# NVIDIA/tensorrt-laboratory

Hardware: NVIDIA H100
Metric: ResNet-50 fp16 b=8 inferences/sec (higher is better)
Workload: dtype f16

## Files before the change

tensorrt_laboratory_b200/csrc/engine.cu:

```cuda
#include <cuda.h>
#include <cuda_runtime.h>
#include <stdarg.h>
#include <stdio.h>
#include <stdlib.h>
#include <string.h>

#include <algorithm>
#include <map>
#include <memory>
#include <mutex>
#include <string>
#include <vector>

#include "../../include/b200infer.h"
#include "kernels.h"
#include "plan_format.h"

#include "b2_internal.h"

namespace b2i {
thread_local std::string g_err;
int fail(int code, const char* fmt, ...) {
    char buf[1024];
    va_list ap;
// ... 697 lines not shown
        const int tiles = m_tiles * (cout_phys / bn);
        for (int splits = 1; splits <= 8; ++splits) {
            if (honor_forced && c->force_splits && !group_span ? splits != c->force_splits : splits != 1) continue;
            if (splits > 1 && (kb != 64 || kblocks / splits < 4 || tiles * splits > 160 || tiles > kMaxSplitTiles ||
                               size_t(tiles) * splits * 128 * bn * 4 > kSplitWorkspaceBytes))
                continue;
            const int kpc = (kblocks + splits - 1) / splits;
            if (splits > 1 && (splits - 1) * kpc >= kblocks) continue;
            for (int st : stgs) {
                if (!b2k::conv_config_exists(bn, kb, st)) continue;
                if (b2k::conv_smem_bytes(bn, st, residual) > kSmemLimit) continue;
                if (honor_forced && c->force_stages && st != c->force_stages) continue;
                if (!(honor_forced && c->force_stages) && !stage_depth_useful(bn, kb, st, kpc)) continue;
                const double smem = b2k::conv_smem_bytes(bn, st, residual);
                int per_sm = int(double(kSmemLimit) / smem);
                per_sm = std::min(per_sm, bn <= 64 ? 2 : 1);
                per_sm = std::max(1, std::min(per_sm, 8));
                const int ctas = tiles * splits;
                const int waves = (ctas + g_sms * per_sm - 1) / (g_sms * per_sm);
                const int sharing = std::max(1, std::min(per_sm, (ctas + g_sms - 1) / g_sms));
                const double stage_bytes = 16384.0 + bn * 128.0;
                const double t_kb = std::max(stage_bytes / (70000.0 / sharing), 1.0 / st);
                double t_epi = 0.6 + bn / 64.0 * 0.4 + (residual ? 0.4 : 0.0);
                if (splits > 1) t_epi += 1.0 + 0.3 * splits;
                const double t_cta = 2.0 + kpc * t_kb + t_epi;
                double total = waves * t_cta;
                const double traffic = double(ctas) * kpc * stage_bytes;
                total = std::max(total, traffic / 5.0e6 + 2.0);
                if (total < best.est_us) best = ConvConfig{bn, st, splits, total};
            }
        }
// ... 1767 lines not shown
```

tensorrt_laboratory_b200/csrc/kernels.cu:

```cuda
#include "kernels.h"

#include <stdio.h>
#include <stdlib.h>
#include <string.h>

#include "ptx_sm90.cuh"
#include "wgmma_sm90.cuh"

namespace b2k {

template <int BN, int STAGES, int SPS = 1>
struct ConvCfg {
    static constexpr int A_SUBBLK = 128 * 64 * 2;
    static constexpr int B_SUBBLK = BN * 64 * 2;
    static constexpr int A_STAGE = SPS * A_SUBBLK;
    static constexpr int B_STAGE = SPS * B_SUBBLK;
    static constexpr int PIPE_BYTES = STAGES * (A_STAGE + B_STAGE);
    static constexpr int TILE_BYTES = 128 * BN * 2;
    static_assert(TILE_BYTES <= PIPE_BYTES, "the output staging tile reuses the pipeline buffers");
};

__host__ __device__ constexpr int conv_smem_layout_bytes(int bn, int stages, bool residual, int sps = 1) {
    return stages * sps * (128 * 64 * 2 + bn * 64 * 2) + (residual ? 128 * bn * 2 : 0) + 256 + bn * 4 + 1024;
}

constexpr int kConvThreads = 384;
constexpr int kConsumerWarps = 8;

struct FragPos {
    int row0, col0;
    __device__ FragPos(int consumer_warp, int lane)
        : row0(64 * (consumer_warp >> 2) + 16 * (consumer_warp & 3) + (lane >> 2)), col0(2 * (lane & 3)) {}
};

template <int BN, int KB, int STAGES, int SPS, int CN = 1, bool DBG = false, int AV = 0, bool GELU = false>
__global__ void __launch_bounds__(kConvThreads, BN <= 64 ? 2 : 1)
conv_f16_tcgen05(const __grid_constant__ CUtensorMap mapA, const __grid_constant__ CUtensorMap mapB,
                 const __grid_constant__ CUtensorMap mapOut, const __grid_constant__ CUtensorMap mapRes,
                 const ConvArgs p) {
    static_assert(SPS == 1 || KB == 64, "multi-sub-block stages exist for the 64-wide K path only");
    using Cfg = ConvCfg<BN, STAGES, SPS>;
    constexpr int TPS = 64 / KB;
    constexpr int A_SUB = 128 * KB * 2;
    constexpr int B_SUB = BN * KB * 2;
    constexpr int OW = BN >= 64 ? 64 : 32;
    constexpr int OROWB = OW * 2;
    constexpr int NBOX = BN / OW;

    extern __shared__ uint8_t smem_raw[];
    uint8_t* smem = smem_raw + ((1024u - (smem_u32(smem_raw) & 1023u)) & 1023u);
    const bool has_res = p.residual != nullptr;
    uint8_t* sA = smem;
    uint8_t* sB = smem + STAGES * Cfg::A_STAGE;
    uint8_t* sOut = smem;
    uint8_t* sRes = smem + Cfg::PIPE_BYTES;
    uint8_t* tail = sRes + (has_res ? Cfg::TILE_BYTES : 0);
// ... 37 lines not shown
    if (threadIdx.x == 0) {
        tma_prefetch_desc(&mapA);
        tma_prefetch_desc(&mapB);
        tma_prefetch_desc(&mapOut);
        if (has_res) tma_prefetch_desc(&mapRes);
        for (int s = 0; s < STAGES; ++s) {
            mbar_init(&full_bar[s], 1);
            mbar_init(&empty_bar[s], static_cast<uint32_t>(kConsumerWarps * cn));
        }
        mbar_init(res_bar, 1);
        fence_barrier_init();
        fence_proxy_async();
    }
    __syncthreads();
    if (cn > 1) cluster_sync_all();
    if (warp == 3) {
#pragma unroll
        for (int i = 0; i < BN / 32; ++i) s_bias[lane + 32 * i] = __ldg(p.bias + n0 + lane + 32 * i);
    }
    if (p.pdl_trigger == 0) pdl_launch_dependents();
    if (dbg && threadIdx.x == 0) dbg[1] = clock64();

    auto sub_tiles = [&](int kb) -> int {
        if (KB == 64) return 1;
        const int n = p.taps_phys - kb * TPS;
        return n > TPS ? TPS : n;
    };
    const bool skip_a = DBG && KB == 64 && (p.dbg_mode & 2), skip_b = DBG && KB == 64 && (p.dbg_mode & 4);
    auto stage_bytes = [&](int kb) -> uint32_t {
        if (KB == 64) {
            const int ns = subs_in_step((kb - kb_begin) / SPS);
            return static_cast<uint32_t>(ns * ((skip_a ? 0 : Cfg::A_SUBBLK) + (skip_b ? 0 : Cfg::B_SUBBLK)));
        }
        return static_cast<uint32_t>(sub_tiles(kb) * (A_SUB + B_SUB));
    };
    auto load_b = [&](int kb, int s) {
// ... 8 lines not shown
                } else {
                    tma_load_2d(&mapB, &full_bar[s], b_dst + u * Cfg::B_SUBBLK, (kb + u) * 64, n0);
                }
            }
        } else {
            const int nt = sub_tiles(kb);
            for (int t = 0; t < nt; ++t) tma_load_2d(&mapB, &full_bar[s], b_dst + t * B_SUB, (kb * TPS + t) * KB, n0);
        }
    };
    auto load_residual = [&]() {
        mbar_expect_tx(res_bar, Cfg::TILE_BYTES);
#pragma unroll
        for (int b = 0; b < NBOX; ++b) tma_load_2d(&mapRes, res_bar, sRes + b * (128 * OROWB), n0 + b * OW, m0);
    };

    if (warp == 0) {
        {
            int img0 = 0, p0 = 0, q0 = 0;
            const int slice_rows = 128 / cn;
            int ms = m0 + static_cast<int>(crank) * slice_rows;
            const uint32_t slice_off = crank * static_cast<uint32_t>(slice_rows) * 128u;
            if (!a_tiled) {
                if (ms >= p.M) ms = 0;
                img0 = ms / p.HoWo;
                const int rem = ms - img0 * p.HoWo;
                p0 = rem / p.Wo;
                q0 = rem - p0 * p.Wo;
            }
            const int base_w = q0 * p.stride_w - p.pad_w;
            const int base_h = p0 * p.stride_h - p.pad_h;
            int cur_cb = 0, cur_r = 0, cur_sx = 0;
            int cb0 = 0;
// ... 68 lines not shown
                if (dbg) c0 = clock64();
                mbar_wait(&empty_bar[s], ph ^ 1);
                if (dbg) c1 = clock64();
                if (elect_one_sync()) {
                    mbar_expect_tx(&full_bar[s], stage_bytes(kb_begin + i * SPS));
                    load_a(kb_begin + i * SPS, s);
                    if (!kSplitProducers) load_b(kb_begin + i * SPS, s);
                }
                __syncwarp();
                if (dbg) {
                    c3 = clock64();
                    tw += c1 - c0, tl += c3 - c1;
                }
            }
            if (dbg && lane == 0) dbg[11] = tw, dbg[12] = te, dbg[13] = tl;
        }
        __syncwarp();
    }

    const int cw = warp - 4;
    float acc[BN / 2];
    if (warp >= 4) {
        const uint32_t wg = static_cast<uint32_t>(cw >> 2);
        auto release_stage = [&](int st) {
            __syncwarp();
            if (lane == 0) {
                if (cn > 1) {
                    for (uint32_t r = 0; r < static_cast<uint32_t>(cn); ++r) mbar_arrive_cluster(&empty_bar[st], r);
                } else {
                    mbar_arrive(&empty_bar[st]);
                }
            }
        };
        long long mw = 0, mi = 0;
        for (int i = 0; i < nk; ++i) {
            const int s = i % STAGES;
            const uint32_t ph = (i / STAGES) & 1;
            long long m0c = 0, m1c = 0;
            if (dbg) m0c = clock64();
            mbar_wait(&full_bar[s], ph);
            if (dbg) m1c = clock64(), mw += m1c - m0c;
            if (dbg && i == 0 && cw == 0 && lane == 0) dbg[3] = clock64();
            const uint32_t a_addr = smem_u32(sA + s * Cfg::A_STAGE);
            const uint32_t b_addr = smem_u32(sB + s * Cfg::B_STAGE);
            if constexpr (KB == 64) {
                auto mma = [&](int t) {
                    const int u = t >> 2, j = t & 3;
                    const uint64_t ad = make_wgmma_desc(a_addr + u * Cfg::A_SUBBLK + wg * 8192 + j * 32, 16, 1024, WG_SW128);
                    const uint64_t bd = make_wgmma_desc(b_addr + u * Cfg::B_SUBBLK + j * 32, 16, 1024, WG_SW128);
                    wgmma_f16<BN>(acc, ad, bd, (i > 0 || t > 0) ? 1u : 0u);
                };
                if (SPS == 1 || subs_in_step(i) == SPS) wgmma_group<4 * SPS>(mma);
                else wgmma_group<4>(mma);
            } else if constexpr (KB == 32) {
                auto mma = [&](int t) {
                    const int st = t >> 1, j = t & 1;
                    const uint64_t ad = make_wgmma_desc(a_addr + st * A_SUB + wg * 4096 + j * 32, 16, 512, WG_SW64);
                    const uint64_t bd = make_wgmma_desc(b_addr + st * B_SUB + j * 32, 16, 512, WG_SW64);
                    wgmma_f16<BN>(acc, ad, bd, (i > 0 || t > 0) ? 1u : 0u);
                };
                if (sub_tiles(kb_begin + i) == TPS) wgmma_group<2 * TPS>(mma);
                else wgmma_group<2>(mma);
            } else {
                auto mma = [&](int j) {
                    const uint64_t ad = make_wgmma_desc(a_addr + 2 * j * A_SUB + wg * 1024, A_SUB, 128, WG_NOSWZ);
                    const uint64_t bd = make_wgmma_desc(b_addr + 2 * j * B_SUB, B_SUB, 128, WG_NOSWZ);
                    wgmma_f16<BN>(acc, ad, bd, (i > 0 || j > 0) ? 1u : 0u);
                };
                wgmma_group_upto<TPS / 2>(sub_tiles(kb_begin + i) / 2, mma);
            }
            if constexpr (STAGES == 1) {
                wgmma_wait<0>();
                release_stage(0);
            } else {
                wgmma_wait<1>();
                if (i > 0) release_stage((i - 1) % STAGES);
            }
            if (dbg) mi += clock64() - m1c;
        }
        if constexpr (STAGES > 1) {
            wgmma_wait<0>();
            if (nk > 0) release_stage((nk - 1) % STAGES);
        }
        if (dbg && cw == 0 && lane == 0) dbg[4] = clock64(), dbg[14] = mw, dbg[15] = mi;
    }

    if (warp == 3 && KB == 64) {
        for (int i = 0; i < nk; ++i) {
            const int s = i % STAGES;
            if (i >= STAGES) mbar_wait(&empty_bar[s], ((i / STAGES) & 1) ^ 1);
            if (elect_one_sync()) load_b(kb_begin + i * SPS, s);
            __syncwarp();
        }
    }

    pdl_wait();
    __syncthreads();
    if (dbg && threadIdx.x == 128) dbg[5] = clock64();
    if (p.pdl_trigger == 1) pdl_launch_dependents();
    const FragPos fp(cw, lane);

    auto finish_pair = [&](int row, int col, float v0, float v1) {
        const int box = col / OW;
        const int chunk = (col % OW) / 8;
        const uint32_t so = static_cast<uint32_t>(box * (128 * OROWB)) + swz_off<OROWB>(row, chunk) + (col % 8) * 2;
        v0 += s_bias[col];
        v1 += s_bias[col + 1];
        if (has_res) {
            const float2 rf = __half22float2(*reinterpret_cast<const __half2*>(sRes + so));
            v0 += rf.x;
            v1 += rf.y;
        }
        if constexpr (GELU) {
            v0 = gelu_erf(v0);
            v1 = gelu_erf(v1);
        } else if (p.relu) {
            v0 = fmaxf(v0, 0.0f);
            v1 = fmaxf(v1, 0.0f);
        }
        *reinterpret_cast<__half2*>(sOut + so) = __floats2half2_rn(v0, v1);
    };

    bool do_store = true;
    if (!split) {
        if (warp >= 4) {
            if (has_res) mbar_wait(res_bar, 0);
#pragma unroll
            for (int j = 0; j < BN / 8; ++j)
#pragma unroll
                for (int h = 0; h < 2; ++h) finish_pair(fp.row0 + 8 * h, 8 * j + fp.col0, acc[4 * j + 2 * h], acc[4 * j + 2 * h + 1]);
        }
    } else {
        const int tile = blockIdx.y * gridDim.x + blockIdx.x;
        float* ws_tile = p.workspace + static_cast<size_t>(tile) * p.splits * (128 * BN);
        if (warp >= 4) {
            float* mine = ws_tile + static_cast<size_t>(blockIdx.z) * (128 * BN);
#pragma unroll
            for (int j = 0; j < BN / 8; ++j)
#pragma unroll
                for (int h = 0; h < 2; ++h)
                    __stcg(reinterpret_cast<float2*>(mine + (fp.row0 + 8 * h) * BN + 8 * j + fp.col0),
                           make_float2(acc[4 * j + 2 * h], acc[4 * j + 2 * h + 1]));
        }
        __syncthreads();
        if (threadIdx.x == 0) {
            __threadfence();
            const int prev = atomicAdd(p.tile_counters + tile, 1);
            const uint32_t last = (prev == p.splits - 1) ? 1u : 0u;
            if (last) {
                p.tile_counters[tile] = 0;
                if (has_res) load_residual();
            }
            *last_flag = last;
        }
        __syncthreads();
        do_store = *last_flag != 0;
        if (do_store && warp >= 4) {
            __threadfence();
            if (has_res) mbar_wait(res_bar, 0);
#pragma unroll 4
            for (int j = 0; j < BN / 8; ++j) {
#pragma unroll
                for (int h = 0; h < 2; ++h) {
                    const int row = fp.row0 + 8 * h, col = 8 * j + fp.col0;
                    float f0 = 0.f, f1 = 0.f;
                    for (int sp = 0; sp < p.splits; ++sp) {
                        const float2 t = __ldcg(reinterpret_cast<const float2*>(ws_tile + static_cast<size_t>(sp) * (128 * BN) + row * BN + col));
                        f0 += t.x;
                        f1 += t.y;
                    }
                    finish_pair(row, col, f0, f1);
                }
            }
        }
    }
    if (dbg && threadIdx.x == 128) dbg[6] = clock64();
    if (p.pdl_trigger == 2) pdl_launch_dependents();
    fence_proxy_async();
    __syncthreads();
    if (threadIdx.x == 0 && do_store) {
#pragma unroll
        for (int b = 0; b < NBOX; ++b) tma_store_2d(&mapOut, sOut + b * (128 * OROWB), n0 + b * OW, m0);
        tma_store_commit_and_wait_read();
    }
    if (cn > 1) {
        if (warp == 1) {
            const int first = nk > STAGES ? nk - STAGES : 0;
            for (int i = first; i < nk; ++i) mbar_wait(&empty_bar[i % STAGES], (i / STAGES) & 1);
        }
        __syncthreads();
        cluster_sync_all();
    }
    if (dbg && threadIdx.x == 128) {
        dbg[7] = clock64();
        unsigned long long gt;
        asm volatile("mov.u64 %0, %%globaltimer;" : "=l"(gt));
        dbg[9] = static_cast<long long>(gt);
    }
}

__host__ __device__ constexpr int conv_ws_smem_bytes(int bn, int stages, int sps, bool residual) {
    return stages * sps * (128 * 64 * 2 + bn * 64 * 2) + 2 * 128 * bn * 2 + (residual ? 2 * 128 * bn * 2 : 0) + 256 + 1024;
}

template <int BN, int STAGES, int SPS>
__global__ void __launch_bounds__(kConvThreads, 1)
conv_f16_tcgen05_ws(const __grid_constant__ CUtensorMap mapA, const __grid_constant__ CUtensorMap mapOut,
                    const __grid_constant__ CUtensorMap mapRes, const ConvArgs p) {
    constexpr int A_SUBBLK = 128 * 64 * 2;
    constexpr int B_SUBBLK = BN * 64 * 2;
    constexpr int A_STAGE = SPS * A_SUBBLK;
    constexpr int B_STAGE = SPS * B_SUBBLK;
// ... 220 lines not shown
}

constexpr int kHaloMaxCBlocks = 8;
__host__ __device__ constexpr int halo_b_stages(int bn) { return bn >= 256 ? 3 : 4; }
__host__ __device__ constexpr int halo_a_stage_bytes(int w, int r) {
    const int loaded = (r + 2) * (w + 2);
    const int touched = 128 + 2 * (w + 2) + 2;
    const int rows = loaded > touched ? loaded : touched;
    return (rows * 128 + 1023) / 1024 * 1024;
}
__host__ __device__ constexpr int halo_smem_bytes(int bn, int w, int r, int cblocks) {
    return cblocks * halo_a_stage_bytes(w, r) + halo_b_stages(bn) * bn * 128 + 256 + bn * 4 + 1024;
}

template <int BN>
__global__ void __launch_bounds__(kConvThreads, 1)
conv3x3_halo_tcgen05(const __grid_constant__ CUtensorMap mapIn, const __grid_constant__ CUtensorMap mapOut, const ConvArgs p) {
    constexpr int NB = halo_b_stages(BN);
    constexpr int B_BLK = BN * 128;
    constexpr int OW = 64;
    constexpr int NBOX = BN / OW;

    extern __shared__ uint8_t smem_raw[];
    uint8_t* smem = smem_raw + ((1024u - (smem_u32(smem_raw) & 1023u)) & 1023u);
    const int W = p.Wo, Wp = p.Wo + 2, R = p.halo_rows;
    const int a_stage = halo_a_stage_bytes(W, R);
    const int cblocks = p.cblocks;
    uint8_t* sA = smem;
    uint8_t* sB = smem + cblocks * a_stage;
    uint8_t* sOut = smem;
    uint8_t* tail = sB + NB * B_BLK;
    uint64_t* a_full = reinterpret_cast<uint64_t*>(tail);
    uint64_t* b_full = a_full + kHaloMaxCBlocks;
// ... 12 lines not shown
    if (threadIdx.x == 0) {
        tma_prefetch_desc(&mapIn);
        tma_prefetch_desc(&mapOut);
        for (int s = 0; s < cblocks; ++s) mbar_init(&a_full[s], 1);
        for (int s = 0; s < NB; ++s) {
            mbar_init(&b_full[s], 1);
            mbar_init(&b_empty[s], kConsumerWarps);
        }
        fence_barrier_init();
        fence_proxy_async();
    }
    __syncthreads();
    if (p.pdl_trigger == 0) pdl_launch_dependents();

    float acc[BN / 2];
    if (warp == 0) {
        const uint32_t halo_bytes = static_cast<uint32_t>((R + 2) * Wp * 128);
        pdl_wait();
        if (elect_one_sync()) {
            for (int cb = 0; cb < cblocks; ++cb) {
                mbar_expect_tx(&a_full[cb], halo_bytes);
                tma_load_4d(&mapIn, &a_full[cb], sA + cb * a_stage, cb * 64, -1, h0 - 1, img);
            }
        }
        __syncwarp();
    } else if (warp >= 4) {
        const uint32_t wg_off = static_cast<uint32_t>((warp - 4) >> 2) * 8192u;
        int i = 0;
#pragma unroll 1
        for (int tap = 0; tap < 9; ++tap) {
            const int r = tap / 3, sx = tap - r * 3;
            const uint32_t tap_off = static_cast<uint32_t>((r * Wp + sx) * 128);
#pragma unroll 1
            for (int cb = 0; cb < cblocks; ++cb, ++i) {
                const int sb = i % NB;
                if (tap == 0) mbar_wait(&a_full[cb], 0);
                mbar_wait(&b_full[sb], (i / NB) & 1);
                const uint32_t a_addr = smem_u32(sA + cb * a_stage) + tap_off + wg_off;
                const uint32_t b_addr = smem_u32(sB + sb * B_BLK);
                wgmma_fence();
#pragma unroll
                for (int j = 0; j < 4; ++j) {
                    const uint64_t ad = make_wgmma_desc(a_addr + j * 32, 16, 1024, WG_SW128);
                    const uint64_t bd = make_wgmma_desc(b_addr + j * 32, 16, 1024, WG_SW128);
                    wgmma_f16<BN>(acc, ad, bd, (i > 0 || j > 0) ? 1u : 0u);
                }
                wgmma_commit();
                wgmma_wait<1>();
                __syncwarp();
                if (i > 0 && lane == 0) mbar_arrive(&b_empty[(i - 1) % NB]);
            }
        }
        wgmma_wait<0>();
        __syncwarp();
        if (lane == 0) mbar_arrive(&b_empty[(nsteps - 1) % NB]);
    } else if (warp == 3) {
        for (int i = lane; i < BN; i += 32) s_bias[i] = __ldg(p.bias + n0 + i);
        for (int i = 0; i < nsteps; ++i) {
            const int sb = i % NB;
            if (i >= NB) mbar_wait(&b_empty[sb], ((i / NB) & 1) ^ 1);
            if (elect_one_sync()) {
                mbar_expect_tx(&b_full[sb], B_BLK);
                bulk_load_1d(&b_full[sb], sB + sb * B_BLK, p.wpacked + (static_cast<size_t>(i) * (p.Cout >> 5) + (n0 >> 5)) * 4096,
                             B_BLK);
            }
            __syncwarp();
        }
    }

    pdl_wait();
    __syncthreads();
    if (p.pdl_trigger == 1) pdl_launch_dependents();
    if (warp >= 4) {
        const FragPos fp(warp - 4, lane);
#pragma unroll
        for (int j = 0; j < BN / 8; ++j) {
#pragma unroll
            for (int h = 0; h < 2; ++h) {
                const int row = fp.row0 + 8 * h, col = 8 * j + fp.col0;
                const uint32_t so = static_cast<uint32_t>((col / OW) * (128 * 128)) + swz_off<128>(row, (col % OW) / 8) + (col % 8) * 2;
                float v0 = acc[4 * j + 2 * h] + s_bias[col], v1 = acc[4 * j + 2 * h + 1] + s_bias[col + 1];
                if (p.relu) {
                    v0 = fmaxf(v0, 0.0f);
                    v1 = fmaxf(v1, 0.0f);
                }
                *reinterpret_cast<__half2*>(sOut + so) = __floats2half2_rn(v0, v1);
            }
        }
    }
    fence_proxy_async();
    __syncthreads();
    if (threadIdx.x == 0) {
#pragma unroll
        for (int b = 0; b < NBOX; ++b) tma_store_4d(&mapOut, sOut + b * (128 * 128), n0 + b * OW, 0, h0, img);
        tma_store_commit_and_wait_read();
    }
}

static bool g_use_pdl = true;
void set_pdl(bool on) { g_use_pdl = on; }
bool get_pdl() { return g_use_pdl; }

template <typename Kern, typename... Args>
static int launch_kernel_cluster(Kern kern, dim3 grid, dim3 block, size_t smem, cudaStream_t stream, bool pdl, unsigned cluster_x,
                                 Args... args) {
    cudaLaunchConfig_t cfg = {};
    cfg.gridDim = grid;
    cfg.blockDim = block;
    cfg.dynamicSmemBytes = smem;
    cfg.stream = stream;
// ... 58 lines not shown
                                                      cudaFuncAttributeMaxDynamicSharedMemorySize, bytes));
        if (e) return e;
        if constexpr (KB == 64) {
            if ((e = static_cast<int>(cudaFuncSetAttribute(conv_f16_tcgen05<BN, KB, STAGES, SPS, 1, false, 1>,
                                                           cudaFuncAttributeMaxDynamicSharedMemorySize, bytes)))) return e;
            if ((e = static_cast<int>(cudaFuncSetAttribute(conv_f16_tcgen05<BN, KB, STAGES, SPS, 1, false, 2>,
                                                           cudaFuncAttributeMaxDynamicSharedMemorySize, bytes)))) return e;
            if ((e = static_cast<int>(cudaFuncSetAttribute(conv_f16_tcgen05<BN, KB, STAGES, SPS, 1, false, 2, true>,
                                                           cudaFuncAttributeMaxDynamicSharedMemorySize, bytes)))) return e;
        }
    }
    return static_cast<int>(cudaFuncSetAttribute(conv_f16_tcgen05<BN, KB, STAGES, SPS, CN>, cudaFuncAttributeMaxDynamicSharedMemorySize, bytes));
}

int conv_smem_bytes(int bn, int stages, bool residual, int sps) { return conv_smem_layout_bytes(bn, stages, residual, sps); }

#define B2_FOR_EACH_CONV(X) \
    X(32, 64, 1, 1) X(32, 64, 2, 1) X(32, 64, 4, 1) X(32, 64, 8, 1) \
    X(64, 64, 1, 1) X(64, 64, 2, 1) X(64, 64, 4, 1) X(64, 64, 8, 1) \
    X(128, 64, 1, 1) X(128, 64, 2, 1) X(128, 64, 4, 1) X(256, 64, 2, 1) X(256, 64, 4, 1) \
    X(32, 64, 2, 2) X(32, 64, 4, 2) X(64, 64, 2, 2) X(64, 64, 4, 2) X(128, 64, 2, 2) X(256, 64, 2, 2) \
    X(32, 8, 2, 1) X(32, 8, 4, 1) X(64, 8, 2, 1) X(64, 8, 4, 1) X(64, 8, 8, 1) X(128, 8, 4, 1) \
    X(32, 32, 2, 1) X(32, 32, 4, 1) X(64, 32, 1, 1) X(64, 32, 2, 1) X(64, 32, 4, 1) X(128, 32, 2, 1) X(128, 32, 4, 1)

int conv_halo_smem(int bn, int w, int r, int cblocks) { return halo_smem_bytes(bn, w, r, cblocks); }
bool conv_halo_config_exists(int bn) { return bn == 64 || bn == 128 || bn == 256; }
static int init_conv_halo_kernels() {
    int e;
    if ((e = static_cast<int>(cudaFuncSetAttribute(conv3x3_halo_tcgen05<64>, cudaFuncAttributeMaxDynamicSharedMemorySize, 227 * 1024)))) return e;
    if ((e = static_cast<int>(cudaFuncSetAttribute(conv3x3_halo_tcgen05<128>, cudaFuncAttributeMaxDynamicSharedMemorySize, 227 * 1024)))) return e;
// ... 906 lines not shown
```

tensorrt_laboratory_b200/csrc/kernels.h:

```cpp
#pragma once
#include <cuda.h>
#include <cuda_fp16.h>
#include <cuda_runtime.h>
#include <stdint.h>

namespace b2k {

enum { A_TILED = 0, A_IM2COL = 1 };

struct ConvArgs {
    const float* bias;
    const __half* residual;
    __half* out;
    int M;
    int Cout;
    int num_kblocks;
    int cblocks;
    int taps;
    int taps_phys;
    int kw;
    int HoWo, Wo;
    int stride_h, stride_w;
    int pad_h, pad_w;
    int relu;
// ... 20 lines not shown
    ConvArgs args;
    int bn;
    int kb;
    int stages;
    int sps;
    int grid_m, grid_n;
    int cn;
    int halo;
    int ws_ctas;
};

int launch_conv_f16_tcgen05(const ConvLaunch& L, cudaStream_t stream);
int init_conv_kernels();
bool conv_config_exists(int bn, int kb, int stages, int sps = 1);
int conv_smem_bytes(int bn, int stages, bool residual, int sps = 1);
bool conv_cluster_config_exists(int bn, int stages, int sps, int cn);
bool conv_halo_config_exists(int bn);
int conv_halo_smem(int bn, int w, int r, int cblocks);
bool conv_ws_config_exists(int bn, int stages, int sps);
int conv_ws_smem(int bn, int stages, int sps, bool residual);
void set_pdl(bool on);
bool get_pdl();

constexpr int kNetMaxLayers = 160;

struct NetLayerInfo {
    const uint8_t* wpacked;
    const float* bias;
    __half* out;
    const __half* residual;
// ... 129 lines not shown
```

tensorrt_laboratory_b200/csrc/ptx_sm90.cuh:

```cuda
#pragma once
#include <cuda.h>
#include <cuda_fp16.h>
#include <cuda_runtime.h>
#include <stdint.h>

namespace b2k {

__device__ __forceinline__ uint32_t smem_u32(const void* p) {
    return static_cast<uint32_t>(__cvta_generic_to_shared(p));
}

__device__ __forceinline__ void mbar_init(uint64_t* bar, uint32_t count) {
    asm volatile("mbarrier.init.shared::cta.b64 [%0], %1;" ::"r"(smem_u32(bar)), "r"(count) : "memory");
}

__device__ __forceinline__ void mbar_expect_tx(uint64_t* bar, uint32_t bytes) {
    asm volatile("mbarrier.arrive.expect_tx.shared::cta.b64 _, [%0], %1;" ::"r"(smem_u32(bar)), "r"(bytes)
                 : "memory");
}

__device__ __forceinline__ uint32_t mbar_try_wait(uint64_t* bar, uint32_t parity) {
    uint32_t ok;
    asm volatile(
        "{\n"
        ".reg .pred p;\n"
        "mbarrier.try_wait.parity.shared::cta.b64 p, [%1], %2;\n"
        "selp.u32 %0, 1, 0, p;\n"
        "}\n"
        : "=r"(ok)
        : "r"(smem_u32(bar)), "r"(parity)
        : "memory");
    return ok;
}

__device__ __forceinline__ void mbar_wait(uint64_t* bar, uint32_t parity) {
    uint32_t spins = 0;
    long long t0 = 0;
    while (!mbar_try_wait(bar, parity)) {
        if ((++spins & 0x3FFFu) == 0) {
            long long now = clock64();
            if (t0 == 0) t0 = now;
            else if (now - t0 > 4000000000LL) __trap();
        }
    }
}

__device__ __forceinline__ bool elect_one_sync() {
    uint32_t pred;
    asm volatile(
        "{\n"
        ".reg .pred P;\n"
        "elect.sync _|P, 0xffffffff;\n"
        "selp.u32 %0, 1, 0, P;\n"
        "}\n"
        : "=r"(pred));
    return pred != 0;
}
// ... 79 lines not shown
}
__device__ __forceinline__ void tma_store_commit() { asm volatile("cp.async.bulk.commit_group;" ::: "memory"); }
__device__ __forceinline__ void tma_store_wait_read0() { asm volatile("cp.async.bulk.wait_group.read 0;" ::: "memory"); }
__device__ __forceinline__ void tma_store_wait_read1() { asm volatile("cp.async.bulk.wait_group.read 1;" ::: "memory"); }
__device__ __forceinline__ void tma_store_commit_and_wait_read() {
    asm volatile("cp.async.bulk.commit_group;" ::: "memory");
    asm volatile("cp.async.bulk.wait_group.read 0;" ::: "memory");
}

template <int ROWB>
__device__ __forceinline__ uint32_t swz_off(int row, int chunk) {
    if (ROWB == 128) return static_cast<uint32_t>(row * 128 + ((chunk ^ (row & 7)) << 4));
    return static_cast<uint32_t>(row * 64 + ((chunk ^ ((row >> 1) & 3)) << 4));
}

__device__ __forceinline__ void named_bar_sync(uint32_t id, uint32_t nthreads) {
    asm volatile("bar.sync %0, %1;" ::"r"(id), "r"(nthreads) : "memory");
}
__device__ __forceinline__ void mbar_arrive(uint64_t* bar) {
    asm volatile("mbarrier.arrive.shared::cta.b64 _, [%0];" ::"r"(smem_u32(bar)) : "memory");
}

__device__ __forceinline__ void tma_load_4d(const CUtensorMap* map, uint64_t* bar, void* dst, int c0, int c1, int c2, int c3) {
    asm volatile(
        "cp.async.bulk.tensor.4d.shared::cluster.global.mbarrier::complete_tx::bytes [%0], [%1, {%3, %4, %5, %6}], [%2];"
        ::"r"(smem_u32(dst)), "l"(reinterpret_cast<uint64_t>(map)), "r"(smem_u32(bar)), "r"(c0), "r"(c1), "r"(c2), "r"(c3)
        : "memory");
}
__device__ __forceinline__ void tma_store_4d(const CUtensorMap* map, const void* src, int c0, int c1, int c2, int c3) {
    asm volatile("cp.async.bulk.tensor.4d.global.shared::cta.bulk_group [%0, {%2, %3, %4, %5}], [%1];" ::"l"(
// ... 7 lines not shown
```

tensorrt_laboratory_b200/csrc/wgmma_sm90.cuh:

```cuda
#pragma once
#include <stdint.h>

namespace b2k {

__device__ __forceinline__ void wgmma_fence() { asm volatile("wgmma.fence.sync.aligned;" ::: "memory"); }
__device__ __forceinline__ void wgmma_commit() { asm volatile("wgmma.commit_group.sync.aligned;" ::: "memory"); }
template <int N>
__device__ __forceinline__ void wgmma_wait() { asm volatile("wgmma.wait_group.sync.aligned %0;" ::"n"(N) : "memory"); }

enum { WG_NOSWZ = 0, WG_SW128 = 1, WG_SW64 = 2 };
__device__ __forceinline__ uint64_t make_wgmma_desc(uint32_t saddr, uint32_t lbo_bytes, uint32_t sbo_bytes, uint32_t layout) {
    uint64_t d = 0;
    d |= static_cast<uint64_t>((saddr >> 4) & 0x3FFF);
    d |= static_cast<uint64_t>((lbo_bytes >> 4) & 0x3FFF) << 16;
    d |= static_cast<uint64_t>((sbo_bytes >> 4) & 0x3FFF) << 32;
    d |= static_cast<uint64_t>(layout & 3) << 62;
    return d;
}

__device__ __forceinline__ void wgmma_f16_n32(float (&d)[16], uint64_t a, uint64_t b, uint32_t accumulate) {
    asm volatile(
        "{\n.reg .pred p;\nsetp.ne.b32 p, %18, 0;\n"
        "wgmma.mma_async.sync.aligned.m64n32k16.f32.f16.f16 {%0, %1, %2, %3, %4, %5, %6, %7, %8, %9, %10, %11, %12, %13, %14, %15}, %16, %17, p, 1, 1, 0, 0;\n}\n"
        : "+f"(d[0]), "+f"(d[1]), "+f"(d[2]), "+f"(d[3]), "+f"(d[4]), "+f"(d[5]), "+f"(d[6]), "+f"(d[7]), "+f"(d[8]), "+f"(d[9]), "+f"(d[10]), "+f"(d[11]), "+f"(d[12]), "+f"(d[13]), "+f"(d[14]), "+f"(d[15])
// ... 43 lines not shown
}
__device__ __forceinline__ void wgmma_i8_n256(int32_t (&d)[128], uint64_t a, uint64_t b, uint32_t accumulate) {
    asm volatile(
        "{\n.reg .pred p;\nsetp.ne.b32 p, %130, 0;\n"
        "wgmma.mma_async.sync.aligned.m64n256k32.s32.s8.s8 {%0, %1, %2, %3, %4, %5, %6, %7, %8, %9, %10, %11, %12, %13, %14, %15, %16, %17, %18, %19, %20, %21, %22, %23, %24, %25, %26, %27, %28, %29, %30, %31, %32, %33, %34, %35, %36, %37, %38, %39, %40, %41, %42, %43, %44, %45, %46, %47, %48, %49, %50, %51, %52, %53, %54, %55, %56, %57, %58, %59, %60, %61, %62, %63, %64, %65, %66, %67, %68, %69, %70, %71, %72, %73, %74, %75, %76, %77, %78, %79, %80, %81, %82, %83, %84, %85, %86, %87, %88, %89, %90, %91, %92, %93, %94, %95, %96, %97, %98, %99, %100, %101, %102, %103, %104, %105, %106, %107, %108, %109, %110, %111, %112, %113, %114, %115, %116, %117, %118, %119, %120, %121, %122, %123, %124, %125, %126, %127}, %128, %129, p;\n}\n"
        : "+r"(d[0]), "+r"(d[1]), "+r"(d[2]), "+r"(d[3]), "+r"(d[4]), "+r"(d[5]), "+r"(d[6]), "+r"(d[7]), "+r"(d[8]), "+r"(d[9]), "+r"(d[10]), "+r"(d[11]), "+r"(d[12]), "+r"(d[13]), "+r"(d[14]), "+r"(d[15]), "+r"(d[16]), "+r"(d[17]), "+r"(d[18]), "+r"(d[19]), "+r"(d[20]), "+r"(d[21]), "+r"(d[22]), "+r"(d[23]), "+r"(d[24]), "+r"(d[25]), "+r"(d[26]), "+r"(d[27]), "+r"(d[28]), "+r"(d[29]), "+r"(d[30]), "+r"(d[31]), "+r"(d[32]), "+r"(d[33]), "+r"(d[34]), "+r"(d[35]), "+r"(d[36]), "+r"(d[37]), "+r"(d[38]), "+r"(d[39]), "+r"(d[40]), "+r"(d[41]), "+r"(d[42]), "+r"(d[43]), "+r"(d[44]), "+r"(d[45]), "+r"(d[46]), "+r"(d[47]), "+r"(d[48]), "+r"(d[49]), "+r"(d[50]), "+r"(d[51]), "+r"(d[52]), "+r"(d[53]), "+r"(d[54]), "+r"(d[55]), "+r"(d[56]), "+r"(d[57]), "+r"(d[58]), "+r"(d[59]), "+r"(d[60]), "+r"(d[61]), "+r"(d[62]), "+r"(d[63]), "+r"(d[64]), "+r"(d[65]), "+r"(d[66]), "+r"(d[67]), "+r"(d[68]), "+r"(d[69]), "+r"(d[70]), "+r"(d[71]), "+r"(d[72]), "+r"(d[73]), "+r"(d[74]), "+r"(d[75]), "+r"(d[76]), "+r"(d[77]), "+r"(d[78]), "+r"(d[79]), "+r"(d[80]), "+r"(d[81]), "+r"(d[82]), "+r"(d[83]), "+r"(d[84]), "+r"(d[85]), "+r"(d[86]), "+r"(d[87]), "+r"(d[88]), "+r"(d[89]), "+r"(d[90]), "+r"(d[91]), "+r"(d[92]), "+r"(d[93]), "+r"(d[94]), "+r"(d[95]), "+r"(d[96]), "+r"(d[97]), "+r"(d[98]), "+r"(d[99]), "+r"(d[100]), "+r"(d[101]), "+r"(d[102]), "+r"(d[103]), "+r"(d[104]), "+r"(d[105]), "+r"(d[106]), "+r"(d[107]), "+r"(d[108]), "+r"(d[109]), "+r"(d[110]), "+r"(d[111]), "+r"(d[112]), "+r"(d[113]), "+r"(d[114]), "+r"(d[115]), "+r"(d[116]), "+r"(d[117]), "+r"(d[118]), "+r"(d[119]), "+r"(d[120]), "+r"(d[121]), "+r"(d[122]), "+r"(d[123]), "+r"(d[124]), "+r"(d[125]), "+r"(d[126]), "+r"(d[127])
        : "l"(a), "l"(b), "r"(accumulate));
}
template <int N>
__device__ __forceinline__ void wgmma_f16(float (&d)[N / 2], uint64_t a, uint64_t b, uint32_t accumulate) {
    if constexpr (N == 32) wgmma_f16_n32(d, a, b, accumulate);
    else if constexpr (N == 64) wgmma_f16_n64(d, a, b, accumulate);
    else if constexpr (N == 128) wgmma_f16_n128(d, a, b, accumulate);
    else wgmma_f16_n256(d, a, b, accumulate);
}
template <int N>
__device__ __forceinline__ void wgmma_i8(int32_t (&d)[N / 2], uint64_t a, uint64_t b, uint32_t accumulate) {
    if constexpr (N == 32) wgmma_i8_n32(d, a, b, accumulate);
    else if constexpr (N == 64) wgmma_i8_n64(d, a, b, accumulate);
    else if constexpr (N == 128) wgmma_i8_n128(d, a, b, accumulate);
    else wgmma_i8_n256(d, a, b, accumulate);
}

template <int N, class F>
__device__ __forceinline__ void wgmma_group(F&& mma) {
    wgmma_fence();
#pragma unroll
    for (int t = 0; t < N; ++t) mma(t);
    wgmma_commit();
}
// ... 13 lines not shown
```

Before: 29970.

## Rebalance warpgroup registers with setmaxnreg and allow two CTAs per SM for BN=128

Producer warpgroups now give up registers with setmaxnreg.dec and consumer warpgroups take more with setmaxnreg.inc, so accumulators can fit when launch bounds ask for two CTAs per SM. BN=128 conv kernels, and BN<=64 halo kernels, get min-blocks 2 when shared memory allows. The host cost model now uses the same CTAs-per-SM rule. When registers are tight, the wgmma N dimension is split into column blocks. The epilogue is moved into a per-role lambda and some barrier waits drop the trap path. The risks are register spills in the consumer warps, and extra wgmma instructions when N is split.

Measured after the change: 30830 (median of 6 runs). +2.9%, better.

```diff
diff --git a/tensorrt_laboratory_b200/csrc/engine.cu b/tensorrt_laboratory_b200/csrc/engine.cu
--- a/tensorrt_laboratory_b200/csrc/engine.cu
+++ b/tensorrt_laboratory_b200/csrc/engine.cu
@@ -735,7 +735,7 @@
                 if (!(honor_forced && c->force_stages) && !stage_depth_useful(bn, kb, st, kpc)) continue;
                 const double smem = b2k::conv_smem_bytes(bn, st, residual);
                 int per_sm = int(double(kSmemLimit) / smem);
-                per_sm = std::min(per_sm, bn <= 64 ? 2 : 1);
+                per_sm = std::min(per_sm, b2k::conv_regs_ctas_per_sm(bn, st));
                 per_sm = std::max(1, std::min(per_sm, 8));
                 const int ctas = tiles * splits;
                 const int waves = (ctas + g_sms * per_sm - 1) / (g_sms * per_sm);
diff --git a/tensorrt_laboratory_b200/csrc/kernels.cu b/tensorrt_laboratory_b200/csrc/kernels.cu
--- a/tensorrt_laboratory_b200/csrc/kernels.cu
+++ b/tensorrt_laboratory_b200/csrc/kernels.cu
@@ -3,6 +3,8 @@
 #include <stdio.h>
 #include <stdlib.h>
 #include <string.h>
+
+#include <type_traits>
 
 #include "ptx_sm90.cuh"
 #include "wgmma_sm90.cuh"
@@ -27,6 +29,19 @@
 constexpr int kConvThreads = 384;
 constexpr int kConsumerWarps = 8;
 
+template <int BN, int MinBlocks>
+struct ConvRegs {
+    static constexpr int kLaunch = 65536 / (kConvThreads * MinBlocks) / 8 * 8;
+    static constexpr int kProducer = 40;
+    static constexpr int kConsumer = (kConvThreads * kLaunch - 128 * kProducer) / 256 / 8 * 8;
+    static constexpr int kMmaN = BN / 2 + 26 <= kLaunch ? BN : 64;
+    static_assert(128 * kProducer + 256 * kConsumer <= kConvThreads * kLaunch, "setmaxnreg.inc would wait forever");
+    static_assert(kConsumer <= 256 && BN / 2 + 32 <= kConsumer, "setmaxnreg range, accumulators");
+};
+__host__ __device__ constexpr int conv_min_blocks(int bn, int stages, int sps) {
+    return bn <= 64 || (bn == 128 && 2 * (conv_smem_layout_bytes(bn, stages, true, sps) + 1024) <= 228 * 1024) ? 2 : 1;
+}
+
 struct FragPos {
     int row0, col0;
     __device__ FragPos(int consumer_warp, int lane)
@@ -34,12 +49,13 @@
 };
 
 template <int BN, int KB, int STAGES, int SPS, int CN = 1, bool DBG = false, int AV = 0, bool GELU = false>
-__global__ void __launch_bounds__(kConvThreads, BN <= 64 ? 2 : 1)
+__global__ void __launch_bounds__(kConvThreads, conv_min_blocks(BN, STAGES, SPS))
 conv_f16_tcgen05(const __grid_constant__ CUtensorMap mapA, const __grid_constant__ CUtensorMap mapB,
                  const __grid_constant__ CUtensorMap mapOut, const __grid_constant__ CUtensorMap mapRes,
                  const ConvArgs p) {
     static_assert(SPS == 1 || KB == 64, "multi-sub-block stages exist for the 64-wide K path only");
     using Cfg = ConvCfg<BN, STAGES, SPS>;
+    using Regs = ConvRegs<BN, conv_min_blocks(BN, STAGES, SPS)>;
     constexpr int TPS = 64 / KB;
     constexpr int A_SUB = 128 * KB * 2;
     constexpr int B_SUB = BN * KB * 2;
@@ -107,12 +123,6 @@
     }
     __syncthreads();
     if (cn > 1) cluster_sync_all();
-    if (warp == 3) {
-#pragma unroll
-        for (int i = 0; i < BN / 32; ++i) s_bias[lane + 32 * i] = __ldg(p.bias + n0 + lane + 32 * i);
-    }
-    if (p.pdl_trigger == 0) pdl_launch_dependents();
-    if (dbg && threadIdx.x == 0) dbg[1] = clock64();
 
     auto sub_tiles = [&](int kb) -> int {
         if (KB == 64) return 1;
@@ -151,8 +161,125 @@
         for (int b = 0; b < NBOX; ++b) tma_load_2d(&mapRes, res_bar, sRes + b * (128 * OROWB), n0 + b * OW, m0);
     };
 
-    if (warp == 0) {
-        {
+    const int cw = warp - 4;
+    float acc[BN / 2];
+
+    auto epilogue = [&](auto role) {
+        constexpr bool kConsumer = decltype(role)::value;
+        pdl_wait();
+        __syncthreads();
+        if (kConsumer && dbg && threadIdx.x == 128) dbg[5] = clock64();
+        if (p.pdl_trigger == 1) pdl_launch_dependents();
+        const FragPos fp(cw, lane);
+
+        auto finish_pair = [&](int row, int col, float v0, float v1) {
+            const int box = col / OW;
+            const int chunk = (col % OW) / 8;
+            const uint32_t so = static_cast<uint32_t>(box * (128 * OROWB)) + swz_off<OROWB>(row, chunk) + (col % 8) * 2;
+            v0 += s_bias[col];
+            v1 += s_bias[col + 1];
+            if (has_res) {
+                const float2 rf = __half22float2(*reinterpret_cast<const __half2*>(sRes + so));
+                v0 += rf.x;
+                v1 += rf.y;
+            }
+            if constexpr (GELU) {
+                v0 = gelu_erf(v0);
+                v1 = gelu_erf(v1);
+            } else if (p.relu) {
+                v0 = fmaxf(v0, 0.0f);
+                v1 = fmaxf(v1, 0.0f);
+            }
+            *reinterpret_cast<__half2*>(sOut + so) = __floats2half2_rn(v0, v1);
+        };
+
+        bool do_store = true;
+        if (!split) {
+            if constexpr (kConsumer) {
+                if (has_res) mbar_wait<false>(res_bar, 0);
+#pragma unroll
+                for (int j = 0; j < BN / 8; ++j)
+#pragma unroll
+                    for (int h = 0; h < 2; ++h) finish_pair(fp.row0 + 8 * h, 8 * j + fp.col0, acc[4 * j + 2 * h], acc[4 * j + 2 * h + 1]);
+            }
+        } else {
+            const int tile = blockIdx.y * gridDim.x + blockIdx.x;
+            float* ws_tile = p.workspace + static_cast<size_t>(tile) * p.splits * (128 * BN);
+            if constexpr (kConsumer) {
+                float* mine = ws_tile + static_cast<size_t>(blockIdx.z) * (128 * BN);
+#pragma unroll
+                for (int j = 0; j < BN / 8; ++j)
+#pragma unroll
+                    for (int h = 0; h < 2; ++h)
+                        __stcg(reinterpret_cast<float2*>(mine + (fp.row0 + 8 * h) * BN + 8 * j + fp.col0),
+                               make_float2(acc[4 * j + 2 * h], acc[4 * j + 2 * h + 1]));
+            }
+            __syncthreads();
+            if (!kConsumer && threadIdx.x == 0) {
+                __threadfence();
+                const int prev = atomicAdd(p.tile_counters + tile, 1);
+                const uint32_t last = (prev == p.splits - 1) ? 1u : 0u;
+                if (last) {
+                    p.tile_counters[tile] = 0;
+                    if (has_res) load_residual();
+                }
+                *last_flag = last;
+            }
+            __syncthreads();
+            do_store = *last_flag != 0;
+            if (kConsumer && do_store) {
+                __threadfence();
+                if (has_res) mbar_wait<false>(res_bar, 0);
+#pragma unroll 4
+                for (int j = 0; j < BN / 8; ++j) {
+#pragma unroll
+                    for (int h = 0; h < 2; ++h) {
+                        const int row = fp.row0 + 8 * h, col = 8 * j + fp.col0;
+                        float f0 = 0.f, f1 = 0.f;
+                        for (int sp = 0; sp < p.splits; ++sp) {
+                            const float2 t = __ldcg(reinterpret_cast<const float2*>(ws_tile + static_cast<size_t>(sp) * (128 * BN) + row * BN + col));
+                            f0 += t.x;
+                            f1 += t.y;
+                        }
+                        finish_pair(row, col, f0, f1);
+                    }
+                }
+            }
+        }
+        if (kConsumer && dbg && threadIdx.x == 128) dbg[6] = clock64();
+        if (p.pdl_trigger == 2) pdl_launch_dependents();
+        fence_proxy_async();
+        __syncthreads();
+        if (!kConsumer && threadIdx.x == 0 && do_store) {
+#pragma unroll
+            for (int b = 0; b < NBOX; ++b) tma_store_2d(&mapOut, sOut + b * (128 * OROWB), n0 + b * OW, m0);
+            tma_store_commit_and_wait_read();
+        }
+        if (cn > 1) {
+            if (!kConsumer && warp == 1) {
+                const int first = nk > STAGES ? nk - STAGES : 0;
+                for (int i = first; i < nk; ++i) mbar_wait(&empty_bar[i % STAGES], (i / STAGES) & 1);
+            }
+            __syncthreads();
+            cluster_sync_all();
+        }
+        if (kConsumer && dbg && threadIdx.x == 128) {
+            dbg[7] = clock64();
+            unsigned long long gt;
+            asm volatile("mov.u64 %0, %%globaltimer;" : "=l"(gt));
+            dbg[9] = static_cast<long long>(gt);
+        }
+    };
+
+    if (warp < 4) {
+        warpgroup_reg_dealloc<Regs::kProducer>();
+        if (warp == 3) {
+#pragma unroll
+            for (int i = 0; i < BN / 32; ++i) s_bias[lane + 32 * i] = __ldg(p.bias + n0 + lane + 32 * i);
+        }
+        if (p.pdl_trigger == 0) pdl_launch_dependents();
+        if (dbg && threadIdx.x == 0) dbg[1] = clock64();
+        if (warp == 0) {
             int img0 = 0, p0 = 0, q0 = 0;
             const int slice_rows = 128 / cn;
             int ms = m0 + static_cast<int>(crank) * slice_rows;
@@ -251,13 +378,20 @@
                 }
             }
             if (dbg && lane == 0) dbg[11] = tw, dbg[12] = te, dbg[13] = tl;
-        }
-        __syncwarp();
-    }
-
-    const int cw = warp - 4;
-    float acc[BN / 2];
-    if (warp >= 4) {
+            __syncwarp();
+        }
+        if (warp == 3 && KB == 64) {
+            for (int i = 0; i < nk; ++i) {
+                const int s = i % STAGES;
+                if (i >= STAGES) mbar_wait(&empty_bar[s], ((i / STAGES) & 1) ^ 1);
+                if (elect_one_sync()) load_b(kb_begin + i * SPS, s);
+                __syncwarp();
+            }
+        }
+        epilogue(std::false_type());
+    } else {
+        warpgroup_reg_alloc<Regs::kConsumer>();
+        if (p.pdl_trigger == 0) pdl_launch_dependents();
         const uint32_t wg = static_cast<uint32_t>(cw >> 2);
         auto release_stage = [&](int st) {
             __syncwarp();
@@ -275,7 +409,7 @@
             const uint32_t ph = (i / STAGES) & 1;
             long long m0c = 0, m1c = 0;
             if (dbg) m0c = clock64();
-            mbar_wait(&full_bar[s], ph);
+            mbar_wait<false>(&full_bar[s], ph);
             if (dbg) m1c = clock64(), mw += m1c - m0c;
             if (dbg && i == 0 && cw == 0 && lane == 0) dbg[3] = clock64();
             const uint32_t a_addr = smem_u32(sA + s * Cfg::A_STAGE);
@@ -284,8 +418,8 @@
                 auto mma = [&](int t) {
                     const int u = t >> 2, j = t & 3;
                     const uint64_t ad = make_wgmma_desc(a_addr + u * Cfg::A_SUBBLK + wg * 8192 + j * 32, 16, 1024, WG_SW128);
-                    const uint64_t bd = make_wgmma_desc(b_addr + u * Cfg::B_SUBBLK + j * 32, 16, 1024, WG_SW128);
-                    wgmma_f16<BN>(acc, ad, bd, (i > 0 || t > 0) ? 1u : 0u);
+                    wgmma_f16_cols<BN, Regs::kMmaN>(acc, ad, b_addr + u * Cfg::B_SUBBLK + j * 32, 16, 1024, WG_SW128, 128,
+                                                    (i > 0 || t > 0) ? 1u : 0u);
                 };
                 if (SPS == 1 || subs_in_step(i) == SPS) wgmma_group<4 * SPS>(mma);
                 else wgmma_group<4>(mma);
@@ -293,16 +427,16 @@
                 auto mma = [&](int t) {
                     const int st = t >> 1, j = t & 1;
                     const uint64_t ad = make_wgmma_desc(a_addr + st * A_SUB + wg * 4096 + j * 32, 16, 512, WG_SW64);
-                    const uint64_t bd = make_wgmma_desc(b_addr + st * B_SUB + j * 32, 16, 512, WG_SW64);
-                    wgmma_f16<BN>(acc, ad, bd, (i > 0 || t > 0) ? 1u : 0u);
+                    wgmma_f16_cols<BN, Regs::kMmaN>(acc, ad, b_addr + st * B_SUB + j * 32, 16, 512, WG_SW64, 64,
+                                                    (i > 0 || t > 0) ? 1u : 0u);
                 };
                 if (sub_tiles(kb_begin + i) == TPS) wgmma_group<2 * TPS>(mma);
                 else wgmma_group<2>(mma);
             } else {
                 auto mma = [&](int j) {
                     const uint64_t ad = make_wgmma_desc(a_addr + 2 * j * A_SUB + wg * 1024, A_SUB, 128, WG_NOSWZ);
-                    const uint64_t bd = make_wgmma_desc(b_addr + 2 * j * B_SUB, B_SUB, 128, WG_NOSWZ);
-                    wgmma_f16<BN>(acc, ad, bd, (i > 0 || j > 0) ? 1u : 0u);
+                    wgmma_f16_cols<BN, Regs::kMmaN>(acc, ad, b_addr + 2 * j * B_SUB, B_SUB, 128, WG_NOSWZ, 16,
+                                                    (i > 0 || j > 0) ? 1u : 0u);
                 };
                 wgmma_group_upto<TPS / 2>(sub_tiles(kb_begin + i) / 2, mma);
             }
@@ -320,119 +454,7 @@
             if (nk > 0) release_stage((nk - 1) % STAGES);
         }
         if (dbg && cw == 0 && lane == 0) dbg[4] = clock64(), dbg[14] = mw, dbg[15] = mi;
-    }
-
-    if (warp == 3 && KB == 64) {
-        for (int i = 0; i < nk; ++i) {
-            const int s = i % STAGES;
-            if (i >= STAGES) mbar_wait(&empty_bar[s], ((i / STAGES) & 1) ^ 1);
-            if (elect_one_sync()) load_b(kb_begin + i * SPS, s);
-            __syncwarp();
-        }
-    }
-
-    pdl_wait();
-    __syncthreads();
-    if (dbg && threadIdx.x == 128) dbg[5] = clock64();
-    if (p.pdl_trigger == 1) pdl_launch_dependents();
-    const FragPos fp(cw, lane);
-
-    auto finish_pair = [&](int row, int col, float v0, float v1) {
-        const int box = col / OW;
-        const int chunk = (col % OW) / 8;
-        const uint32_t so = static_cast<uint32_t>(box * (128 * OROWB)) + swz_off<OROWB>(row, chunk) + (col % 8) * 2;
-        v0 += s_bias[col];
-        v1 += s_bias[col + 1];
-        if (has_res) {
-            const float2 rf = __half22float2(*reinterpret_cast<const __half2*>(sRes + so));
-            v0 += rf.x;
-            v1 += rf.y;
-        }
-        if constexpr (GELU) {
-            v0 = gelu_erf(v0);
-            v1 = gelu_erf(v1);
-        } else if (p.relu) {
-            v0 = fmaxf(v0, 0.0f);
-            v1 = fmaxf(v1, 0.0f);
-        }
-        *reinterpret_cast<__half2*>(sOut + so) = __floats2half2_rn(v0, v1);
-    };
-
-    bool do_store = true;
-    if (!split) {
-        if (warp >= 4) {
-            if (has_res) mbar_wait(res_bar, 0);
-#pragma unroll
-            for (int j = 0; j < BN / 8; ++j)
-#pragma unroll
-                for (int h = 0; h < 2; ++h) finish_pair(fp.row0 + 8 * h, 8 * j + fp.col0, acc[4 * j + 2 * h], acc[4 * j + 2 * h + 1]);
-        }
-    } else {
-        const int tile = blockIdx.y * gridDim.x + blockIdx.x;
-        float* ws_tile = p.workspace + static_cast<size_t>(tile) * p.splits * (128 * BN);
-        if (warp >= 4) {
-            float* mine = ws_tile + static_cast<size_t>(blockIdx.z) * (128 * BN);
-#pragma unroll
-            for (int j = 0; j < BN / 8; ++j)
-#pragma unroll
-                for (int h = 0; h < 2; ++h)
-                    __stcg(reinterpret_cast<float2*>(mine + (fp.row0 + 8 * h) * BN + 8 * j + fp.col0),
-                           make_float2(acc[4 * j + 2 * h], acc[4 * j + 2 * h + 1]));
-        }
-        __syncthreads();
-        if (threadIdx.x == 0) {
-            __threadfence();
-            const int prev = atomicAdd(p.tile_counters + tile, 1);
-            const uint32_t last = (prev == p.splits - 1) ? 1u : 0u;
-            if (last) {
-                p.tile_counters[tile] = 0;
-                if (has_res) load_residual();
-            }
-            *last_flag = last;
-        }
-        __syncthreads();
-        do_store = *last_flag != 0;
-        if (do_store && warp >= 4) {
-            __threadfence();
-            if (has_res) mbar_wait(res_bar, 0);
-#pragma unroll 4
-            for (int j = 0; j < BN / 8; ++j) {
-#pragma unroll
-                for (int h = 0; h < 2; ++h) {
-                    const int row = fp.row0 + 8 * h, col = 8 * j + fp.col0;
-                    float f0 = 0.f, f1 = 0.f;
-                    for (int sp = 0; sp < p.splits; ++sp) {
-                        const float2 t = __ldcg(reinterpret_cast<const float2*>(ws_tile + static_cast<size_t>(sp) * (128 * BN) + row * BN + col));
-                        f0 += t.x;
-                        f1 += t.y;
-                    }
-                    finish_pair(row, col, f0, f1);
-                }
-            }
-        }
-    }
-    if (dbg && threadIdx.x == 128) dbg[6] = clock64();
-    if (p.pdl_trigger == 2) pdl_launch_dependents();
-    fence_proxy_async();
-    __syncthreads();
-    if (threadIdx.x == 0 && do_store) {
-#pragma unroll
-        for (int b = 0; b < NBOX; ++b) tma_store_2d(&mapOut, sOut + b * (128 * OROWB), n0 + b * OW, m0);
-        tma_store_commit_and_wait_read();
-    }
-    if (cn > 1) {
-        if (warp == 1) {
-            const int first = nk > STAGES ? nk - STAGES : 0;
-            for (int i = first; i < nk; ++i) mbar_wait(&empty_bar[i % STAGES], (i / STAGES) & 1);
-        }
-        __syncthreads();
-        cluster_sync_all();
-    }
-    if (dbg && threadIdx.x == 128) {
-        dbg[7] = clock64();
-        unsigned long long gt;
-        asm volatile("mov.u64 %0, %%globaltimer;" : "=l"(gt));
-        dbg[9] = static_cast<long long>(gt);
+        epilogue(std::true_type());
     }
 }
 
@@ -683,9 +705,10 @@
 }
 
 template <int BN>
-__global__ void __launch_bounds__(kConvThreads, 1)
+__global__ void __launch_bounds__(kConvThreads, BN <= 64 ? 2 : 1)
 conv3x3_halo_tcgen05(const __grid_constant__ CUtensorMap mapIn, const __grid_constant__ CUtensorMap mapOut, const ConvArgs p) {
     constexpr int NB = halo_b_stages(BN);
+    using Regs = ConvRegs<BN, BN <= 64 ? 2 : 1>;
     constexpr int B_BLK = BN * 128;
     constexpr int OW = 64;
     constexpr int NBOX = BN / OW;
@@ -728,17 +751,65 @@
     if (p.pdl_trigger == 0) pdl_launch_dependents();
 
     float acc[BN / 2];
-    if (warp == 0) {
-        const uint32_t halo_bytes = static_cast<uint32_t>((R + 2) * Wp * 128);
+    auto epilogue = [&](auto role) {
+        constexpr bool kConsumer = decltype(role)::value;
         pdl_wait();
-        if (elect_one_sync()) {
-            for (int cb = 0; cb < cblocks; ++cb) {
-                mbar_expect_tx(&a_full[cb], halo_bytes);
-                tma_load_4d(&mapIn, &a_full[cb], sA + cb * a_stage, cb * 64, -1, h0 - 1, img);
-            }
-        }
-        __syncwarp();
-    } else if (warp >= 4) {
+        __syncthreads();
+        if (p.pdl_trigger == 1) pdl_launch_dependents();
+        if constexpr (kConsumer) {
+            const FragPos fp(warp - 4, lane);
+#pragma unroll
+            for (int j = 0; j < BN / 8; ++j) {
+#pragma unroll
+                for (int h = 0; h < 2; ++h) {
+                    const int row = fp.row0 + 8 * h, col = 8 * j + fp.col0;
+                    const uint32_t so = static_cast<uint32_t>((col / OW) * (128 * 128)) + swz_off<128>(row, (col % OW) / 8) + (col % 8) * 2;
+                    float v0 = acc[4 * j + 2 * h] + s_bias[col], v1 = acc[4 * j + 2 * h + 1] + s_bias[col + 1];
+                    if (p.relu) {
+                        v0 = fmaxf(v0, 0.0f);
+                        v1 = fmaxf(v1, 0.0f);
+                    }
+                    *reinterpret_cast<__half2*>(sOut + so) = __floats2half2_rn(v0, v1);
+                }
+            }
+        }
+        fence_proxy_async();
+        __syncthreads();
+        if (!kConsumer && threadIdx.x == 0) {
+#pragma unroll
+            for (int b = 0; b < NBOX; ++b) tma_store_4d(&mapOut, sOut + b * (128 * 128), n0 + b * OW, 0, h0, img);
+            tma_store_commit_and_wait_read();
+        }
+    };
+
+    if (warp < 4) {
+        warpgroup_reg_dealloc<Regs::kProducer>();
+        if (warp == 0) {
+            const uint32_t halo_bytes = static_cast<uint32_t>((R + 2) * Wp * 128);
+            pdl_wait();
+            if (elect_one_sync()) {
+                for (int cb = 0; cb < cblocks; ++cb) {
+                    mbar_expect_tx(&a_full[cb], halo_bytes);
+                    tma_load_4d(&mapIn, &a_full[cb], sA + cb * a_stage, cb * 64, -1, h0 - 1, img);
+                }
+            }
+            __syncwarp();
+        } else if (warp == 3) {
+            for (int i = lane; i < BN; i += 32) s_bias[i] = __ldg(p.bias + n0 + i);
+            for (int i = 0; i < nsteps; ++i) {
+                const int sb = i % NB;
+                if (i >= NB) mbar_wait(&b_empty[sb], ((i / NB) & 1) ^ 1);
+                if (elect_one_sync()) {
+                    mbar_expect_tx(&b_full[sb], B_BLK);
+                    bulk_load_1d(&b_full[sb], sB + sb * B_BLK, p.wpacked + (static_cast<size_t>(i) * (p.Cout >> 5) + (n0 >> 5)) * 4096,
+                                 B_BLK);
+                }
+                __syncwarp();
+            }
+        }
+        epilogue(std::false_type());
+    } else {
+        warpgroup_reg_alloc<Regs::kConsumer>();
         const uint32_t wg_off = static_cast<uint32_t>((warp - 4) >> 2) * 8192u;
         int i = 0;
 #pragma unroll 1
@@ -748,8 +819,8 @@
 #pragma unroll 1
             for (int cb = 0; cb < cblocks; ++cb, ++i) {
                 const int sb = i % NB;
-                if (tap == 0) mbar_wait(&a_full[cb], 0);
-                mbar_wait(&b_full[sb], (i / NB) & 1);
+                if (tap == 0) mbar_wait<false>(&a_full[cb], 0);
+                mbar_wait<false>(&b_full[sb], (i / NB) & 1);
                 const uint32_t a_addr = smem_u32(sA + cb * a_stage) + tap_off + wg_off;
                 const uint32_t b_addr = smem_u32(sB + sb * B_BLK);
                 wgmma_fence();
@@ -768,46 +839,7 @@
         wgmma_wait<0>();
         __syncwarp();
         if (lane == 0) mbar_arrive(&b_empty[(nsteps - 1) % NB]);
-    } else if (warp == 3) {
-        for (int i = lane; i < BN; i += 32) s_bias[i] = __ldg(p.bias + n0 + i);
-        for (int i = 0; i < nsteps; ++i) {
-            const int sb = i % NB;
-            if (i >= NB) mbar_wait(&b_empty[sb], ((i / NB) & 1) ^ 1);
-            if (elect_one_sync()) {
-                mbar_expect_tx(&b_full[sb], B_BLK);
-                bulk_load_1d(&b_full[sb], sB + sb * B_BLK, p.wpacked + (static_cast<size_t>(i) * (p.Cout >> 5) + (n0 >> 5)) * 4096,
-                             B_BLK);
-            }
-            __syncwarp();
-        }
-    }
-
-    pdl_wait();
-    __syncthreads();
-    if (p.pdl_trigger == 1) pdl_launch_dependents();
-    if (warp >= 4) {
-        const FragPos fp(warp - 4, lane);
-#pragma unroll
-        for (int j = 0; j < BN / 8; ++j) {
-#pragma unroll
-            for (int h = 0; h < 2; ++h) {
-                const int row = fp.row0 + 8 * h, col = 8 * j + fp.col0;
-                const uint32_t so = static_cast<uint32_t>((col / OW) * (128 * 128)) + swz_off<128>(row, (col % OW) / 8) + (col % 8) * 2;
-                float v0 = acc[4 * j + 2 * h] + s_bias[col], v1 = acc[4 * j + 2 * h + 1] + s_bias[col + 1];
-                if (p.relu) {
-                    v0 = fmaxf(v0, 0.0f);
-                    v1 = fmaxf(v1, 0.0f);
-                }
-                *reinterpret_cast<__half2*>(sOut + so) = __floats2half2_rn(v0, v1);
-            }
-        }
-    }
-    fence_proxy_async();
-    __syncthreads();
-    if (threadIdx.x == 0) {
-#pragma unroll
-        for (int b = 0; b < NBOX; ++b) tma_store_4d(&mapOut, sOut + b * (128 * 128), n0 + b * OW, 0, h0, img);
-        tma_store_commit_and_wait_read();
+        epilogue(std::true_type());
     }
 }
 
@@ -896,6 +928,7 @@
 }
 
 int conv_smem_bytes(int bn, int stages, bool residual, int sps) { return conv_smem_layout_bytes(bn, stages, residual, sps); }
+int conv_regs_ctas_per_sm(int bn, int stages, int sps) { return conv_min_blocks(bn, stages, sps); }
 
 #define B2_FOR_EACH_CONV(X) \
     X(32, 64, 1, 1) X(32, 64, 2, 1) X(32, 64, 4, 1) X(32, 64, 8, 1) \
diff --git a/tensorrt_laboratory_b200/csrc/kernels.h b/tensorrt_laboratory_b200/csrc/kernels.h
--- a/tensorrt_laboratory_b200/csrc/kernels.h
+++ b/tensorrt_laboratory_b200/csrc/kernels.h
@@ -58,6 +58,7 @@
 int init_conv_kernels();
 bool conv_config_exists(int bn, int kb, int stages, int sps = 1);
 int conv_smem_bytes(int bn, int stages, bool residual, int sps = 1);
+int conv_regs_ctas_per_sm(int bn, int stages, int sps = 1);
 bool conv_cluster_config_exists(int bn, int stages, int sps, int cn);
 bool conv_halo_config_exists(int bn);
 int conv_halo_smem(int bn, int w, int r, int cblocks);
diff --git a/tensorrt_laboratory_b200/csrc/ptx_sm90.cuh b/tensorrt_laboratory_b200/csrc/ptx_sm90.cuh
--- a/tensorrt_laboratory_b200/csrc/ptx_sm90.cuh
+++ b/tensorrt_laboratory_b200/csrc/ptx_sm90.cuh
@@ -33,14 +33,19 @@
     return ok;
 }
 
+template <bool kTrap = true>
 __device__ __forceinline__ void mbar_wait(uint64_t* bar, uint32_t parity) {
     uint32_t spins = 0;
     long long t0 = 0;
     while (!mbar_try_wait(bar, parity)) {
         if ((++spins & 0x3FFFu) == 0) {
             long long now = clock64();
-            if (t0 == 0) t0 = now;
-            else if (now - t0 > 4000000000LL) __trap();
+            if (t0 == 0) {
+                t0 = now;
+            } else if (now - t0 > 4000000000LL) {
+                if constexpr (kTrap) __trap();
+                else *reinterpret_cast<volatile int*>(0) = 0;
+            }
         }
     }
 }
@@ -150,6 +155,15 @@
     return static_cast<uint32_t>(row * 64 + ((chunk ^ ((row >> 1) & 3)) << 4));
 }
 
+template <uint32_t N>
+__device__ __forceinline__ void warpgroup_reg_dealloc() {
+    asm volatile("setmaxnreg.dec.sync.aligned.u32 %0;" ::"n"(N));
+}
+template <uint32_t N>
+__device__ __forceinline__ void warpgroup_reg_alloc() {
+    asm volatile("setmaxnreg.inc.sync.aligned.u32 %0;" ::"n"(N));
+}
+
 __device__ __forceinline__ void named_bar_sync(uint32_t id, uint32_t nthreads) {
     asm volatile("bar.sync %0, %1;" ::"r"(id), "r"(nthreads) : "memory");
 }
diff --git a/tensorrt_laboratory_b200/csrc/wgmma_sm90.cuh b/tensorrt_laboratory_b200/csrc/wgmma_sm90.cuh
--- a/tensorrt_laboratory_b200/csrc/wgmma_sm90.cuh
+++ b/tensorrt_laboratory_b200/csrc/wgmma_sm90.cuh
@@ -81,6 +81,16 @@
     else if constexpr (N == 128) wgmma_f16_n128(d, a, b, accumulate);
     else wgmma_f16_n256(d, a, b, accumulate);
 }
+template <int N, int NI>
+__device__ __forceinline__ void wgmma_f16_cols(float (&d)[N / 2], uint64_t a, uint32_t b_addr, uint32_t b_lbo, uint32_t b_sbo,
+                                               uint32_t b_layout, uint32_t b_row, uint32_t accumulate) {
+    static_assert(N % NI == 0, "column blocks tile N");
+#pragma unroll
+    for (int c = 0; c < N / NI; ++c)
+        wgmma_f16<NI>(*reinterpret_cast<float(*)[NI / 2]>(d + c * (NI / 2)), a,
+                      make_wgmma_desc(b_addr + c * NI * b_row, b_lbo, b_sbo, b_layout), accumulate);
+}
+
 template <int N>
 __device__ __forceinline__ void wgmma_i8(int32_t (&d)[N / 2], uint64_t a, uint64_t b, uint32_t accumulate) {
     if constexpr (N == 32) wgmma_i8_n32(d, a, b, accumulate);
```
